# Iancic/Physically-Based-Ray-Tracer

Measured on AMD Instinct MI355X. Metric: Mrays/s (closest-hit segments + shadow any-hit rays) at 1920x1080, 4 spp, depth 4, higher is better.
Workload: dtype f32; 1 GPU; c4-heightfield1m: 1000000 tris, 1920x1080, 4 spp, depth 4; global_batch=2073600, seq_len=4, parallelism=single-gpu, outputs=device (HBM-resident), frames_in_flight=2, warmup_steps_run=75, hw_queues=4

## Files before the change

### include/prt.h

```cpp
#ifndef PRT_H
#define PRT_H
#include <stdint.h>
#include <stddef.h>

#ifdef __cplusplus
extern "C" {
#endif

#define PRT_ABI_VERSION 10

typedef enum {
    PRT_OK = 0,
    PRT_ERR_INVALID_ARGUMENT = -1,
    PRT_ERR_NO_DEVICE = -2,
    PRT_ERR_HIP = -3,
    PRT_ERR_OUT_OF_MEMORY = -4,
    PRT_ERR_NOT_READY = -5,
    PRT_ERR_UNSUPPORTED = -6
} prt_status;

#define PRT_FLAG_AA          (1u << 0)
#define PRT_FLAG_ACCUMULATE  (1u << 1)
#define PRT_FLAG_GAMMA       (1u << 2)
#define PRT_FLAG_NORMALMAP   (1u << 3)
// ... 128 lines not shown
    float vignette_intensity;
    float vignette_radius;
    float color_grading[4];
} prt_postfx;
int prt_postfx_preset(int32_t preset, prt_postfx* out);
int prt_set_postfx(prt_ctx* ctx, const prt_postfx* pfx);

#define PRT_OUT_DEVICE (1u << 0)
int prt_render(prt_ctx* ctx, const prt_render_params* params, float* avg_rgba, uint32_t* rgb8,
               uint32_t out_flags, prt_stats* stats);
int prt_reset_accumulation(prt_ctx* ctx, int32_t full);
int prt_ray_totals(prt_ctx* ctx, uint64_t* segments, uint64_t* shadow_rays, int32_t reset);
int prt_primary_rays(prt_ctx* ctx, uint64_t* traced, uint64_t* reused, int32_t reset);
int prt_shadow_reuse(prt_ctx* ctx, uint64_t* reused, int32_t reset);
int prt_shadow_dead(prt_ctx* ctx, uint64_t* dead, int32_t reset);

int prt_accumulation_bytes(prt_ctx* ctx, uint64_t* bytes);
int prt_save_accumulation(prt_ctx* ctx, void* blob, uint64_t bytes);
int prt_load_accumulation(prt_ctx* ctx, const void* blob, uint64_t bytes);

#define PRT_SHARD_ID_BYTES 128
int prt_shard_unique_id(uint8_t id[PRT_SHARD_ID_BYTES]);
int prt_shard_init_rccl(prt_ctx* ctx, const uint8_t id[PRT_SHARD_ID_BYTES], int32_t rank, int32_t world,
                        int32_t tile_size);
int prt_shard_attach_rccl(prt_ctx* ctx, void* nccl_comm, int32_t tile_size);
int prt_create_group(const prt_device_desc* devices, int32_t count, int32_t tile_size, prt_ctx** out);
typedef struct {
    int32_t rank, world, tile_size;
    int32_t transport;
} prt_shard_info;
// ... 143 lines not shown
```

### include/prt_renderer.hpp

```cpp
#pragma once
#include <algorithm>
#include <array>
#include <cstdint>
#include <map>
#include <stdexcept>
#include <string>
#include <utility>
#include <vector>

#include "prt.h"

namespace prt {

class Error : public std::runtime_error {
 public:
  Error(int code, const std::string& what) : std::runtime_error(what), code(code) {}
  int code;
};

inline void check(int rc) {
  if (rc != PRT_OK) throw Error(rc, std::string("prt error ") + std::to_string(rc) + ": " + prt_last_error());
}

struct Model {
// ... 285 lines not shown
  void RayTotals(uint64_t* segments, uint64_t* shadow_rays, bool reset = false) const {
    check(prt_ray_totals(ctx_, segments, shadow_rays, reset ? 1 : 0));
  }
  void PrimaryRays(uint64_t* traced, uint64_t* reused, bool reset = false) const {
    check(prt_primary_rays(ctx_, traced, reused, reset ? 1 : 0));
  }
  uint64_t ShadowReuse(bool reset = false) const {
    uint64_t reused = 0;
    check(prt_shadow_reuse(ctx_, &reused, reset ? 1 : 0));
    return reused;
  }
  uint64_t ShadowDead(bool reset = false) const {
    uint64_t dead = 0;
    check(prt_shadow_dead(ctx_, &dead, reset ? 1 : 0));
    return dead;
  }

  void Aov(std::vector<float>& albedo, std::vector<float>& normal_depth) {
    albedo.assign(4 * (size_t)width_ * height_, 0.0f);
    normal_depth.assign(4 * (size_t)width_ * height_, 0.0f);
    const prt_postfx pf = camera.PostFx(isPostProcessed);
    check(prt_set_postfx(ctx_, &pf));
    check(prt_render_aov(ctx_, width_, height_, NORMALMAPPED ? PRT_FLAG_NORMALMAP : 0u, albedo.data(),
                         normal_depth.data(), 0u));
  }
  static prt_denoise_params DenoiseDefaults() {
    prt_denoise_params p{};
    check(prt_denoise_defaults(&p));
    return p;
  }
// ... 176 lines not shown
```

### physically-based-ray-tracer_amd/csrc/prt_api_render.cpp

```cpp
#include <hip/hip_runtime.h>

#include <algorithm>
#include <cstdio>
#include <cstdlib>
#include <cstring>
#include <string>
#include <vector>

#include "prt_ctx.h"

using namespace prt;
using namespace prt::host;

namespace {

int check_params(const prt_render_params* p) {
  if (!p) return fail(PRT_ERR_INVALID_ARGUMENT, "params is NULL");
  if (p->width <= 0 || p->height <= 0 || p->width > 16384 || p->height > 16384)
    return fail(PRT_ERR_INVALID_ARGUMENT, "bad resolution");
  if (p->spp < 0) return fail(PRT_ERR_INVALID_ARGUMENT, "spp < 0");
  if ((p->flags & PRT_FLAG_AA) && (p->spp % 2) != 0)
    return fail(PRT_ERR_INVALID_ARGUMENT, "with PRT_FLAG_AA spp must be even (2 paths per reference frame)");
  if (p->bounces < 0 || p->bounces > 16) return fail(PRT_ERR_INVALID_ARGUMENT, "bounces must be in [0,16]");
  if (p->render_mode < 0 || p->render_mode > 6) return fail(PRT_ERR_INVALID_ARGUMENT, "bad render_mode");
// ... 172 lines not shown
    A.frame_index = p->frame_index + f0;
    A.frames = Fb;
    const uint64_t nb = per * (uint64_t)Fb;
    float4* frames = flight_frames(c, fl).as<float4>();
    rc = ensure_wave(ws0, (uint32_t)nb, p->bounces, P.ext(), P.merge(), !P.defer());
    if (rc) return rc;
    ws0.wb.base = 0;
    ws0.wb.coop_tail = P.coop_tail ? 1 : 0;
    ws0.wb.tl = tl;
    ws0.wb.phit = ws0.phit.as<float4>();
    ws0.wb.pitems = (uint32_t)per;
    ws0.wb.pmode = kPrimTrace;
    ws0.wb.lvis = nullptr;
    ws0.wb.lslot = iters + 1;
    ws0.wb.dead = P.dead;
    if (P.preuse && nb > 0) {
      const PrimKey key = prim_key(c, S, M);
      const uint64_t px = tile_image_pixels(M);
      if (ws0.pvalid && std::memcmp(&ws0.pkey, &key, sizeof(key)) == 0) {
        ws0.wb.pmode = kPrimReuse;
        c->prim_reused += px * (uint64_t)Fb;
        if (P.lreuse) {
          float lp[18];
          std::memcpy(lp, S.ppos, sizeof(S.ppos));
          std::memcpy(lp + 12, S.dpos, sizeof(S.dpos));
          std::memcpy(lp + 15, S.spos, sizeof(S.spos));
          if (!(ws0.lvalid && ws0.lgen == ws0.pgen && std::memcmp(lp, ws0.lpos, sizeof(lp)) == 0)) {
            ws0.lvalid = false;
            HIP_TRY(hipMemsetAsync(ws0.lvis.p, 0, sizeof(uint2) * (size_t)per, st));
            ws0.lgen = ws0.pgen;
            std::memcpy(ws0.lpos, lp, sizeof(lp));
            ws0.lvalid = true;
          }
          ws0.wb.lvis = ws0.lvis.as<uint2>();
        }
      } else {
        ws0.wb.pmode = kPrimDense;
        ws0.pgen++;
        ws0.pkey = key;
        ws0.pvalid = false;
        c->prim_traced += px;
        c->prim_reused += px * (uint64_t)(Fb - 1);
      }
    }
    {
      const size_t qw = (size_t)(iters + 2) * 2 * kNSub * kCtrStride;
      const size_t fbase = (size_t)(kMaxIters + 2) * 2 * kNSub * kCtrStride;
      const size_t fw = (size_t)(iters + 2) * 2 * kParts * kCtrStride;
      HIP_TRY(launch_clear2(Lw, ws0.wb.ctr, (uint32_t)qw, ws0.wb.ctr + fbase, (uint32_t)fw));
    }
    if (P.ext() && S.has_diel) HIP_TRY(hipMemsetAsync(ws0.wb.dst, 0, 4ull * ws0.wb.n, st));
    WaveBufs wb = ws0.wb;
    if (P.defer()) point_planes(wb, ws0.planes, (uint32_t)nb, iters);
    HIP_TRY(launch_wave_init(Lw, S, A, M, wb, frames));
    const bool lrec = wb.pmode == kPrimReuse && wb.lvis != nullptr;
    for (uint32_t it = 0; it <= iters; it++)
      HIP_TRY(launch_wave2_iter(Lw, S, A, M, wb, frames, timers ? &c->wt : nullptr, P, lrec, it));
    if (ws0.wb.pmode == kPrimDense) ws0.pvalid = true;
    if (last && want_stats) HIP_TRY(hipEventRecord(c->ev[1], st));
    float4* acc_prev = nullptr;
    if (post && last) {
      const size_t np = (size_t)p->width * p->height;
      if (!avg_dev) { HIP_TRY(c->avg.ensure(np * 16)); avg_dev = c->avg.as<float4>(); }
      if (c->pfx.aberration != 0) { HIP_TRY(c->accprev.ensure(np * 16)); acc_prev = c->accprev.as<float4>(); }
    }
    if (acc_after) HIP_TRY(hipStreamWaitEvent(st, acc_after, 0));
    HIP_TRY(launch_accumulate(L, M, Fb, p->flags, frames, c->acc.as<float4>(), c->nsamp.as<int32_t>(),
                              c->dist.as<float>(), avg_dev, post ? nullptr : rgb8_dev, tiles_dev, acc_prev,
                              ws0.wb.ctr, iters, ray_totals_dev(c)));
    if (post && last) {
      const float4* acc_new = (p->flags & PRT_FLAG_ACCUMULATE) ? c->acc.as<float4>() : avg_dev;
      HIP_TRY(launch_postfx(L, post_params(c, p->width, p->height), acc_new, acc_prev, c->nsamp.as<int32_t>(),
// ... 389 lines not shown

int prt_primary_rays(prt_ctx* c, uint64_t* traced, uint64_t* reused, int32_t reset) {
  if (!c || !traced || !reused) return fail(PRT_ERR_INVALID_ARGUMENT, "bad primary ray counter arguments");
  uint64_t t = c->prim_traced, r = c->prim_reused;
  if (reset) c->prim_traced = c->prim_reused = 0;
  for (prt_ctx* m : c->members) {
    t += m->prim_traced;
    r += m->prim_reused;
    if (reset) m->prim_traced = m->prim_reused = 0;
  }
  *traced = t;
  *reused = r;
  return PRT_OK;
}

int prt_shadow_reuse(prt_ctx* c, uint64_t* reused, int32_t reset) {
  if (!c || !reused) return fail(PRT_ERR_INVALID_ARGUMENT, "bad shadow reuse counter arguments");
  PRT_JOIN(c);
  std::vector<prt_ctx*> all{c};
  all.insert(all.end(), c->members.begin(), c->members.end());
  uint64_t n = 0;
  for (prt_ctx* m : all) {
    HIP_TRY(hipSetDevice(m->device));
    unsigned long long h = 0;
    void* dev = ray_totals_dev(m) + 1;
    HIP_TRY(hipMemcpyAsync(&h, dev, sizeof(h), hipMemcpyDeviceToHost, m->stream));
    if (reset) HIP_TRY(hipMemsetAsync(dev, 0, sizeof(h), m->stream));
    HIP_TRY(hipStreamSynchronize(m->stream));
    n += h;
  }
// ... 180 lines not shown
```

### physically-based-ray-tracer_amd/csrc/prt_ctx.h

```cpp
#pragma once
#include <hip/hip_runtime.h>

#include <memory>
#include <string>
#include <utility>
#include <vector>

#include "../../include/prt.h"
#include "prt_blas_refit_gpu.h"
#include "prt_launch.h"
#include "prt_rccl.h"
#include "prt_refit.h"
#include "prt_skin_gpu.h"
#include "prt_tlas_worker.h"

namespace prt::host {

int fail(int code, const std::string& msg);
std::string& last_error();

#define HIP_TRY(expr)                                                                        \
  do {                                                                                       \
    hipError_t e_ = (expr);                                                                  \
    if (e_ != hipSuccess)                                                                    \
// ... 155 lines not shown
  prt_postfx pfx{};
  DevBuf accprev;
  DevBuf acc, nsamp, dist;
  int32_t accW = 0, accH = 0;
  DevBuf frames, avg, rgb8, counters, hits, tl;
  hipEvent_t ev[3] = {nullptr, nullptr, nullptr};
  prt::host::WaveState ws;
  prt::WaveTimers wt = {};
  uint32_t last_iters = 0;
  bool last_defer = false;
  bool last_timers = false;
  uint64_t last_paths = 0;
  uint64_t carry_segments = 0, carry_shadow = 0;
  uint64_t scene_epoch = 0, inst_epoch = 0;
  uint64_t prim_traced = 0, prim_reused = 0;
  int32_t sh_kind = 0;
  int32_t sh_rank = 0, sh_world = 1, sh_tile = 32;
  ncclComm_t comm = nullptr;
  bool own_comm = false;
  std::vector<prt_ctx*> members;
  DevBuf shtiles, gathered;
  hipEvent_t sh_ev = nullptr;
  bool layout_checked = false;
  int32_t inflight = 1;
  prt::host::Flight fl[prt::host::kMaxFlights];
  int32_t next_fl = 0, last_fl = -1;
  hipEvent_t fl_fork = nullptr;
  DevBuf aov_hits, aov_alb, aov_nd;
  DevBuf dn_in[3], dn_geo, dn_pp[2], dn_out, dn_rgb8;
  hipEvent_t dn_ev[2 + PRT_DENOISE_TIMINGS] = {};
// ... 64 lines not shown
```

### physically-based-ray-tracer_amd/csrc/prt_defer.hip

```cpp
#include "prt_shade2.h"

namespace prt {

template <bool I0>
__global__ void __launch_bounds__(kBlock, I0 ? 4 : 1) k_shade2d(SceneDev S, TraceArgs A, TileMap M, WaveBufs B, uint32_t iter) {
  shade2_body<false, I0, true>(S, A, M, B, iter);
}

__device__ __forceinline__ V3 resolve_path(const SceneDev& S, const WaveBufs& B, uint32_t item, uint32_t first,
                                           uint32_t last, uint32_t rl, uint32_t fl) {
  V3 L = resolve_segment(S, B, (size_t)last * B.n + item, rl, fl);
  for (uint32_t k = last; k > first; k--) {
    const size_t e = (size_t)(k - 1u) * B.n + item;
    const V3 Rk = resolve_segment(S, B, e, B.rinfo[e], fl);
    const float4 Tk = B.T[e];
    L = Rk + L * v3(Tk.x, Tk.y, Tk.z);
  }
  return L;
}
__device__ __forceinline__ uint32_t path_end(const WaveBufs& B, uint32_t item, uint32_t iters, uint32_t it, uint32_t& r) {
  while (((r >> 16) & 3u) == kStNeeCont && it + 1u < iters) r = B.rinfo[(size_t)(++it) * B.n + item];
  return it;
}
template <bool LEARN>
// ... 9 lines not shown
    }
    const uint32_t e1 = path_end(B, item, iters, 0u, r);
    const V3 L1 = resolve_path(S, B, item, 0u, e1, r, fl);
    V3 L = L1;
    if (fl & kAA) {
      if (!(r & kRiQueued) || e1 + 1u >= iters) continue;
      r = B.rinfo[(size_t)(e1 + 1u) * B.n + item];
      const uint32_t e2 = path_end(B, item, iters, e1 + 1u, r);
      L = resolve_path(S, B, item, e1 + 1u, e2, r, fl);
    }
    const V3 res = pixel_value(L1, L, fl);
    out[item] = make_float4(res.x, res.y, res.z, B.s1[item].w);
  }
}

void launch_shade2d(hipStream_t s, unsigned grid, const SceneDev& S, const TraceArgs& A, const TileMap& M,
                    const WaveBufs& B, uint32_t it, bool i0) {
  if (i0) hipLaunchKernelGGL(k_shade2d<true>, dim3(grid), dim3(kBlock), 0, s, S, A, M, B, it);
  else hipLaunchKernelGGL(k_shade2d<false>, dim3(grid), dim3(kBlock), 0, s, S, A, M, B, it);
}
void launch_resolve_pass(hipStream_t s, unsigned grid, const SceneDev& S, const TraceArgs& A, const WaveBufs& B,
                         uint32_t iters, float4* out, bool learn) {
  if (learn) hipLaunchKernelGGL(k_resolve_pass<true>, dim3(grid), dim3(kBlock), 0, s, S, A, B, iters, out);
  else hipLaunchKernelGGL(k_resolve_pass<false>, dim3(grid), dim3(kBlock), 0, s, S, A, B, iters, out);
}

}
```

### physically-based-ray-tracer_amd/csrc/prt_launch.h

```cpp
#pragma once
#include <hip/hip_runtime.h>

#include <cstddef>

#include "prt_kernels.h"
#include "prt_plan.h"
#include "prt_post.h"
#include "prt_traverse8.h"

namespace prt {

struct Counters {
  unsigned long long segments, shadow;
};
struct HitOut {
  float t, u, v;
  uint32_t prim, inst;
};
struct LaunchCfg {
  hipStream_t stream;
  int occ;
  uint32_t groups = 1;
};

// ... 46 lines not shown
void lane_stats_dump();
#endif
constexpr int kTlWaves = 256 * 4 * 8;
struct WaveTimers {
  hipEvent_t ev[4 * (kMaxIters + 1)];
  uint32_t iters;
};

hipError_t launch_wave_init(const LaunchCfg& c, const SceneDev& S, const TraceArgs& A, const TileMap& M,
                            const WaveBufs& B, float4* out);
hipError_t launch_wave2_iter(const LaunchCfg& c, const SceneDev& S, const TraceArgs& A, const TileMap& M,
                             const WaveBufs& B, float4* out, WaveTimers* tm, const WavePlan& P, bool lrec,
                             uint32_t it);
void launch_shade2d(hipStream_t s, unsigned grid, const SceneDev& S, const TraceArgs& A, const TileMap& M,
                    const WaveBufs& B, uint32_t it, bool i0);
void launch_resolve_pass(hipStream_t s, unsigned grid, const SceneDev& S, const TraceArgs& A, const WaveBufs& B,
                         uint32_t iters, float4* out, bool learn);
hipError_t launch_clear2(const LaunchCfg& c, uint32_t* a, uint32_t na, uint32_t* b, uint32_t nb);
hipError_t launch_accumulate(const LaunchCfg& c, const TileMap& M, int32_t frames, uint32_t flags, const float4* fr,
                             float4* acc, int32_t* nsamp, float* dist, float4* avg, uint32_t* rgb8, float4* tiles,
                             float4* acc_prev, const uint32_t* ctr, uint32_t iters, Counters* totals);
hipError_t launch_postfx(const LaunchCfg& c, const PostDev& P, const float4* acc_new, const float4* acc_old,
                         const int32_t* nsamp, const float4* avg, uint32_t* rgb8);
hipError_t launch_untile(const LaunchCfg& c, int32_t W, int32_t H, int32_t ts, int32_t world, uint32_t per_rank,
                         const float4* gathered, float4* avg, uint32_t* rgb8, const PostDev* post);
struct InstSrc;
constexpr uint32_t kSpillTraceBlocks = 256u * 4u * 4u;
constexpr int kSpillTraceStack = 18;
hipError_t launch_refit(hipStream_t s, const InstSrc* src, int32_t n, InstDev* out);
hipError_t launch_wait_host(hipStream_t s, uint32_t* flag, uint32_t* err, double seconds);
// ... 9 lines not shown
```

### physically-based-ray-tracer_amd/csrc/prt_plan.h

```cpp
#pragma once
#include <algorithm>
#include <cassert>
#include <cstddef>
#include <cstdint>
#include <cstdlib>
#include <cstring>

#include "../../include/prt.h"

namespace prt {

constexpr uint32_t kNSub = 32;
constexpr uint32_t kCtrStride = 32;
constexpr uint32_t kParts = 8;
constexpr int kMaxIters = 128;
enum : int32_t { kPrimTrace = 0, kPrimDense = 1, kPrimReuse = 2 };

constexpr uint64_t kMaxPassItems = 1ull << 27;
constexpr uint64_t kMaxMergedPassItems = 1ull << 26;

inline bool debug_queues_on() { return std::getenv("PRT_DEBUG_QUEUES") != nullptr; }
struct Tunables {
  int32_t merge = -1;
  bool defer = true;
  uint64_t defer_budget = 4096ull << 20;
  bool primary_reuse = true;
  bool shadow_reuse = true;
  uint32_t dead_shadow = 2;
  uint64_t max_items = 0;
  bool coop_tail = true;
  bool debug_queues = false;
  int32_t fail_rank = -1;
  bool fail_all = false;
};
inline Tunables read_tunables() {
  Tunables t;
  auto off = [](const char* name) {
    const char* e = std::getenv(name);
    return e && std::atoi(e) == 0;
  };
  if (const char* e = std::getenv("PRT_MERGE")) t.merge = std::atoi(e) != 0 ? 1 : 0;
  t.defer = !off("PRT_DEFER_RESOLVE");
  if (const char* e = std::getenv("PRT_DEFER_BUDGET_MB")) t.defer_budget = std::strtoull(e, nullptr, 10) << 20;
  t.primary_reuse = !off("PRT_PRIMARY_REUSE");
  t.shadow_reuse = !off("PRT_SHADOW_REUSE");
  if (const char* e = std::getenv("PRT_DEAD_SHADOW")) {
    const int v = std::atoi(e);
    t.dead_shadow = v == 0 ? 0u : (v == 1 ? 1u : 2u);
  }
  if (const char* e = std::getenv("PRT_MAX_ITEMS")) t.max_items = std::max<uint64_t>(std::strtoull(e, nullptr, 10), 1);
  t.coop_tail = !off("PRT_TAIL");
  t.debug_queues = debug_queues_on();
  if (const char* e = std::getenv("PRT_FAIL_RENDER"); e && *e) {
    t.fail_all = std::strcmp(e, "all") == 0;
    t.fail_rank = std::max(std::atoi(e), -1);
  }
  return t;
}

constexpr size_t round256(size_t bytes) { return (bytes + 255) & ~size_t(255); }

constexpr size_t kCtrWords = (size_t)(kMaxIters + 2) * 2 * (kNSub + kParts) * kCtrStride;
constexpr uint32_t shadow_per_item(bool merge) { return merge ? 8u : 5u; }

#define PRT_WAVE_ARRAYS(X)                                                                                      \
  X(seed, 4, n, true) X(info, 4, n, true) X(rinfo, 4, ns, true) X(ro, 16, n, true) X(rd, 16, n, true)          \
// ... 53 lines not shown
  const uint32_t paths = (flags & PRT_FLAG_AA) ? 2u : 1u;
  if (merge && paths == 2 && bounces > 0) return 2u * (uint32_t)bounces - 1u;
  if (!dielectric) return paths * (uint32_t)bounces;
  return bounces > 8 ? 0xFFFFFFFFu : paths * ((1u << bounces) - 1u);
}

enum class Pipeline { Plain, PlainDeferred, Merged, Ext, Debug };
struct WavePlan {
  Pipeline pipeline = Pipeline::Plain;
  uint32_t iters = 0;
  int32_t F = 0, fmax = 1, npass = 1, F0 = 0;
  uint64_t per = 0;
  bool preuse = false, lreuse = false;
  uint32_t dead = 2;
  bool coop_tail = true;
  bool timeline = false;
  bool ext() const { return pipeline == Pipeline::Ext; }
  bool merge() const { return pipeline == Pipeline::Merged; }
  bool defer() const { return pipeline == Pipeline::PlainDeferred; }
  uint32_t items0() const { return (uint32_t)(per * (uint64_t)F0); }
};

inline int plan_render(int32_t render_mode, uint32_t flags, int32_t bounces, int32_t spp, uint64_t per, bool area,
                       bool diel, const Tunables& t, WavePlan& P, const char*& err) {
  P = WavePlan{};
  if (per > kMaxPassItems) {
    err = "more than 2^27 pixels in one frame of one shard";
    return PRT_ERR_UNSUPPORTED;
  }
  const bool aa = (flags & PRT_FLAG_AA) != 0;
// ... 13 lines not shown
  P.F0 = std::min(F, P.fmax);
  P.iters = wave_iters(diel, bounces, flags, merge);
  if (P.iters > (uint32_t)kMaxIters) {
    err = diel ? "dielectric path trees exceed the wavefront iteration limit (lower bounces)"
               : "too many wavefront iterations";
    return PRT_ERR_UNSUPPORTED;
  }
  const bool defer = plain && !merge && P.items0() != 0 && t.defer &&
                     plane_layout(P.items0(), P.iters).bytes <= t.defer_budget;
  P.pipeline = merge ? Pipeline::Merged : !mode0 ? Pipeline::Debug : ext ? Pipeline::Ext
               : defer ? Pipeline::PlainDeferred : Pipeline::Plain;
  P.preuse = plain && t.primary_reuse && per > 0 && F > 0;
  P.lreuse = P.preuse && t.shadow_reuse;
  P.dead = t.dead_shadow;
  P.coop_tail = t.coop_tail;
  P.timeline = t.debug_queues;
  return PRT_OK;
}

enum class Kernel {
  None,
  Trace2, Trace2Dense,
  Res2d, Res2dLearn, Res2md, Res2mdLearn,
  ResolvePass, ResolvePassLearn,
  Miss2, Miss2Ext, ResMiss2, ResMiss2Ext,
  Shade2, Shade2Learn, Shade2Ext, Shade2Debug,
  Shade2d, Shade2dLearn, Shade2m, Shade2mLearn,
};
struct Schedule {
  Kernel trace, resolve, shade;
};
inline Schedule wave_schedule(Pipeline p, bool lrec, int32_t pmode, uint32_t it, uint32_t iters) {
  const bool plainish = p == Pipeline::Plain || p == Pipeline::PlainDeferred;
  assert(!lrec || pmode == kPrimReuse);
  assert((plainish || p == Pipeline::Merged) || (pmode == kPrimTrace && !lrec));
  const bool learn_res = lrec && it == 1, learn_shade = lrec && it == 0;
  Schedule s{Kernel::Trace2, Kernel::None, Kernel::None};
  if (it == 0 && pmode == kPrimDense) s.trace = Kernel::Trace2Dense;
  else if (it == 0 && pmode == kPrimReuse && plainish) s.trace = Kernel::None;
  switch (p) {
    case Pipeline::Plain:
      if (it > 0) s.resolve = learn_res ? Kernel::Res2dLearn : Kernel::Res2d;
      s.shade = learn_shade ? Kernel::Shade2Learn : Kernel::Shade2;
      break;
    case Pipeline::PlainDeferred:
      if (it == iters) s.resolve = lrec ? Kernel::ResolvePassLearn : Kernel::ResolvePass;
      s.shade = learn_shade ? Kernel::Shade2dLearn : Kernel::Shade2d;
      break;
    case Pipeline::Merged:
      if (it > 0) s.resolve = learn_res ? Kernel::Res2mdLearn : Kernel::Res2md;
      s.shade = learn_shade ? Kernel::Shade2mLearn : Kernel::Shade2m;
      break;
    case Pipeline::Ext:
      s.resolve = it > 0 ? Kernel::ResMiss2Ext : Kernel::Miss2Ext;
      s.shade = Kernel::Shade2Ext;
      break;
    case Pipeline::Debug:
      s.resolve = it > 0 ? Kernel::ResMiss2 : Kernel::Miss2;
      s.shade = Kernel::Shade2Debug;
      break;
  }
  if (it >= iters) s.shade = Kernel::None;
  return s;
}

}
```

### physically-based-ray-tracer_amd/csrc/prt_wave2.hip

```cpp
#include <cstdio>

#include "prt_launch.h"
#include "prt_path.h"
#include "prt_persist.h"
#include "prt_queue.h"

namespace prt {

#ifdef PRT_LANE_STATS
__device__ unsigned long long g_lane_stats[(kMaxIters + 2) * 32];
void lane_stats_dump() {
  static unsigned long long h[(kMaxIters + 2) * 32];
  if (hipMemcpyFromSymbol(h, HIP_SYMBOL(g_lane_stats), sizeof(h)) != hipSuccess) return;
  for (int i = 0; i < kMaxIters + 2; i++) {
    const unsigned long long* r = h + 32 * i;
    if (!r[31]) continue;
    std::fprintf(stderr, "prt: lanestats %d", i);
    for (int k = 0; k < 32; k++) std::fprintf(stderr, " %llu", r[k]);
    std::fprintf(stderr, "\n");
  }
  static const unsigned long long z[(kMaxIters + 2) * 32] = {};
  (void)hipMemcpyToSymbol(HIP_SYMBOL(g_lane_stats), z, sizeof(z));
}
#endif
// ... 454 lines not shown
  return g < kNSub ? kNSub : g - g % kNSub;
}

hipError_t launch_wave2_iter(const LaunchCfg& c, const SceneDev& S, const TraceArgs& A, const TileMap& M,
                             const WaveBufs& B, float4* out, WaveTimers* tm, const WavePlan& P, bool lrec,
                             uint32_t it) {
  if (B.n == 0) return hipSuccess;
  const unsigned gprod = producer_blocks(c);
#ifndef PRT_SHADE_GRID
  const unsigned gshade = B.n >= (1u << 21) ? 4u * gprod : gprod;
#else
  static_assert(PRT_SHADE_GRID % kNSub == 0, "PRT_SHADE_GRID must be a multiple of kNSub");
  const unsigned gshade = PRT_SHADE_GRID;
#endif
  const uint32_t iters = P.iters;
  const Schedule k = wave_schedule(P.pipeline, lrec, B.pmode, it, iters);
  if (tm) (void)hipEventRecord(tm->ev[4 * it + 0], c.stream);
  WaveBufs Bt = B, Bs = B;
  if (P.defer()) {
    if (it > 0) Bt.vis = B.vis + (size_t)(it - 1u) * B.n;
    const size_t o = (size_t)it * B.n;
    Bs.rinfo += o; Bs.ne += o; Bs.nb += o; Bs.nk += o; Bs.vis += o; Bs.T += o;
  }
  if (k.trace == Kernel::Trace2Dense) launch_trace2_t<true>(c, S, Bt, it, iters);
  else if (k.trace == Kernel::Trace2) launch_trace2_t<false>(c, S, Bt, it, iters);
  if (tm) (void)hipEventRecord(tm->ev[4 * it + 1], c.stream);
#ifndef PRT_RES_GRID
  const unsigned gres = gprod;
#else
  const unsigned gres = PRT_RES_GRID;
#endif
// ... 5 lines not shown
    case Kernel::Res2dLearn: PRT_LAUNCH(k_res2d<true>, gdense, S, A, B, out); break;
    case Kernel::Res2d: PRT_LAUNCH(k_res2d<false>, gdense, S, A, B, out); break;
    case Kernel::ResolvePassLearn: launch_resolve_pass(c.stream, gdense, S, A, B, iters, out, true); break;
    case Kernel::ResolvePass: launch_resolve_pass(c.stream, gdense, S, A, B, iters, out, false); break;
    case Kernel::ResMiss2Ext: PRT_LAUNCH(k_resmiss2<true>, gres, S, A, B, it, iters, 1u, out); break;
    case Kernel::ResMiss2: PRT_LAUNCH(k_resmiss2<false>, gres, S, A, B, it, iters, 1u, out); break;
    case Kernel::Miss2Ext: PRT_LAUNCH(k_miss2<true>, gprod, S, A, B, it); break;
    case Kernel::Miss2: PRT_LAUNCH(k_miss2<false>, gprod, S, A, B, it); break;
    default: assert(k.resolve == Kernel::None);
  }
  switch (k.shade) {
    case Kernel::Shade2mLearn: PRT_LAUNCH(k_shade2m<true>, gshade, S, A, M, B, it); break;
    case Kernel::Shade2m: PRT_LAUNCH(k_shade2m<false>, gshade, S, A, M, B, it); break;
    case Kernel::Shade2Debug: PRT_LAUNCH(k_shade2_debug, gprod, S, A, M, B, it); break;
    case Kernel::Shade2Ext: PRT_LAUNCH(k_shade2<true>, gshade, S, A, M, B, it); break;
    case Kernel::Shade2dLearn: launch_shade2d(c.stream, gshade, S, A, M, Bs, it, true); break;
    case Kernel::Shade2d: launch_shade2d(c.stream, gshade, S, A, M, Bs, it, false); break;
    case Kernel::Shade2Learn: PRT_LAUNCH((k_shade2<false, true>), gshade, S, A, M, B, it); break;
    case Kernel::Shade2: PRT_LAUNCH(k_shade2<false>, gshade, S, A, M, B, it); break;
    default: assert(k.shade == Kernel::None);
  }
#undef PRT_LAUNCH
  if (tm) tm->iters = iters + 1;
  return hipGetLastError();
}

hipError_t launch_wave_init(const LaunchCfg& c, const SceneDev& S, const TraceArgs& A, const TileMap& M,
                            const WaveBufs& B, float4* out) {
  hipLaunchKernelGGL(k_wave_init, dim3(producer_blocks(c)), dim3(kBlock), 0, c.stream, S, A, M, B, out);
  return hipGetLastError();
// ... 4 lines not shown
```

### physically-based-ray-tracer_amd/prt/_lib.py

```python
from __future__ import annotations

import ctypes as C
import os

HERE = os.path.dirname(os.path.abspath(__file__))
LIBPATH = os.environ.get("PRT_LIBPATH") or os.path.join(HERE, "libprt.so")

PRT_OK = 0
ABI_VERSION = 10
FLAG_AA, FLAG_ACCUMULATE, FLAG_GAMMA, FLAG_NORMALMAP, FLAG_SKYBOX, FLAG_LIGHTED, FLAG_STOCHASTIC = (1 << i for i in range(7))
FLAGS_DEFAULT = 0x7F
OUT_DEVICE = 1
IN_DEVICE = 1
OUT_TIMED = 2
DENOISE_TIMINGS = 10
BUILDER_HOST_SAH, BUILDER_GPU_LBVH, BUILDER_HOST_SBVH, BUILDER_GPU_PLOC = 0, 1, 2, 3

MODE_BRDF, MODE_BASECOLOR, MODE_GEOMETRYNORMAL, MODE_SHADINGNORMAL, MODE_METAL, MODE_ROUGHNESS, MODE_EMISSIVE = range(7)

EXPORTS = [
    "prt_abi_version", "prt_last_error", "prt_device_count", "prt_create", "prt_destroy", "prt_set_stream",
    "prt_set_textures", "prt_set_meshes", "prt_set_instances", "prt_set_lights", "prt_set_sky", "prt_set_camera",
    "prt_camera_look_at", "prt_postfx_preset", "prt_set_postfx", "prt_render", "prt_reset_accumulation", "prt_tile_buffer_pixels", "prt_tile_pixel_map",
    "prt_render_tiles",
    "prt_untile", "prt_trace_primary", "prt_intersect", "prt_occluded", "prt_brdf_probe", "prt_get_scene_info", "prt_set_bvh_builder",
    "prt_set_instance_materials", "prt_set_area_lights", "prt_shard_unique_id", "prt_shard_init_rccl",
    "prt_shard_attach_rccl", "prt_create_group", "prt_get_shard_info", "prt_accumulation_bytes",
    "prt_save_accumulation", "prt_load_accumulation", "prt_ray_totals", "prt_set_frames_in_flight", "prt_finish",
    "prt_render_aov", "prt_denoise_defaults", "prt_denoise", "prt_denoise_timings",
    "prt_reproject_defaults", "prt_reproject", "prt_primary_rays", "prt_shadow_reuse",
    "prt_shadow_dead",
    "prt_render_aov_ids", "prt_instance_motion", "prt_reproject_motion",
    "prt_temporal_defaults", "prt_reproject_moments", "prt_denoise_variance_defaults", "prt_denoise_variance",
    "prt_update_mesh", "prt_read_blas", "prt_read_blas_tris",
    "prt_snapshot_mesh", "prt_render_aov_deform", "prt_reproject_deform",
    "prt_set_mesh_skin", "prt_skin_mesh",
]
SHARD_ID_BYTES = 128
SHARD_NONE, SHARD_RCCL, SHARD_GROUP = 0, 1, 2

MAT_TEXTURED, MAT_DIELECTRIC, MAT_MIRROR = 0, 1, 2


class PrtError(RuntimeError):
    pass


class DeviceDesc(C.Structure):
    _fields_ = [("device", C.c_int32), ("flags", C.c_uint32)]


class Texture(C.Structure):
# ... 118 lines not shown
        "prt_set_lights": ([vp, C.POINTER(Lights)], C.c_int),
        "prt_set_sky": ([vp, vp, i32, i32], C.c_int),
        "prt_set_camera": ([vp, C.POINTER(CameraDesc)], C.c_int),
        "prt_camera_look_at": ([vp, vp, C.c_float, C.POINTER(CameraDesc)], C.c_int),
        "prt_postfx_preset": ([i32, C.POINTER(PostFx)], C.c_int),
        "prt_set_postfx": ([vp, C.POINTER(PostFx)], C.c_int),
        "prt_render": ([vp, C.POINTER(RenderParams), vp, vp, u32, C.POINTER(Stats)], C.c_int),
        "prt_reset_accumulation": ([vp, i32], C.c_int),
        "prt_accumulation_bytes": ([vp, C.POINTER(C.c_uint64)], C.c_int),
        "prt_save_accumulation": ([vp, vp, C.c_uint64], C.c_int),
        "prt_load_accumulation": ([vp, vp, C.c_uint64], C.c_int),
        "prt_ray_totals": ([vp, C.POINTER(C.c_uint64), C.POINTER(C.c_uint64), C.c_int32], C.c_int),
        "prt_primary_rays": ([vp, C.POINTER(C.c_uint64), C.POINTER(C.c_uint64), C.c_int32], C.c_int),
        "prt_shadow_reuse": ([vp, C.POINTER(C.c_uint64), C.c_int32], C.c_int),
        "prt_shadow_dead": ([vp, C.POINTER(C.c_uint64), C.c_int32], C.c_int),
        "prt_tile_buffer_pixels": ([i32, i32, i32, i32, C.POINTER(C.c_int64)], C.c_int),
        "prt_tile_pixel_map": ([i32, i32, i32, i32, i32, C.c_void_p], C.c_int),
        "prt_render_tiles": ([vp, C.POINTER(RenderParams), i32, i32, i32, vp, C.POINTER(Stats)], C.c_int),
        "prt_untile": ([vp, vp, i32, i32, i32, i32, vp, vp], C.c_int),
        "prt_trace_primary": ([vp, i32, i32, vp, u32, C.POINTER(Stats)], C.c_int),
        "prt_intersect": ([vp, i32, vp, vp, vp, vp], C.c_int),
        "prt_occluded": ([vp, i32, vp, vp, vp, vp], C.c_int),
        "prt_brdf_probe": ([vp, i32, i32, vp, vp], C.c_int),
        "prt_get_scene_info": ([vp, C.POINTER(SceneInfo)], C.c_int),
        "prt_set_bvh_builder": ([vp, i32], C.c_int),
        "prt_set_instance_materials": ([vp, vp, i32], C.c_int),
        "prt_set_area_lights": ([vp, C.POINTER(AreaLight), i32], C.c_int),
        "prt_shard_unique_id": ([vp], C.c_int),
        "prt_shard_init_rccl": ([vp, vp, i32, i32, i32], C.c_int),
        "prt_shard_attach_rccl": ([vp, vp, i32], C.c_int),
# ... 9 lines not shown
        "prt_render_aov_ids": ([vp, i32, i32, u32, vp, vp, vp, u32], C.c_int),
        "prt_instance_motion": ([vp, vp, i32, vp], C.c_int),
        "prt_reproject_motion": ([vp, C.POINTER(ReprojectParams), i32, i32, C.POINTER(CameraDesc), vp, vp, vp,
                                  C.POINTER(CameraDesc), vp, vp, vp, vp, i32, vp, vp, u32], C.c_int),
        "prt_temporal_defaults": ([C.POINTER(TemporalParams)], C.c_int),
        "prt_reproject_moments": ([vp, C.POINTER(TemporalParams), i32, i32, C.POINTER(CameraDesc), vp, vp, vp,
                                   C.POINTER(CameraDesc), vp, vp, vp, vp, i32, vp, vp, vp, vp, u32], C.c_int),
        "prt_render_aov_deform": ([vp, i32, i32, u32, vp, vp, vp, vp, u32], C.c_int),
        "prt_reproject_deform": ([vp, C.POINTER(TemporalParams), i32, i32, C.POINTER(CameraDesc), vp, vp, vp,
                                  C.POINTER(CameraDesc), vp, vp, vp, vp, i32, vp, vp, vp, vp, vp, vp, u32], C.c_int),
        "prt_denoise_variance_defaults": ([C.POINTER(DenoiseVarianceParams)], C.c_int),
        "prt_denoise_variance": ([vp, C.POINTER(DenoiseVarianceParams), i32, i32, vp, vp, vp, vp, vp, vp, vp, u32],
                                 C.c_int),
    }
    for name, (args, res) in sig.items():
        f = getattr(L, name)
        f.argtypes = args
        f.restype = res
    if L.prt_abi_version() != ABI_VERSION:
        raise PrtError(f"{LIBPATH}: ABI {L.prt_abi_version()} != {ABI_VERSION} (stale build: rerun __graft_entry__.build())")
    _lib = L
    return L


def check(rc: int) -> None:
    if rc != PRT_OK:
        msg = load().prt_last_error()
        raise PrtError(f"prt error {rc}: {msg.decode() if msg else ''}")
```

### physically-based-ray-tracer_amd/prt/renderer.py

```python
from __future__ import annotations

import ctypes as C
from dataclasses import dataclass, field

import numpy as np

from . import _lib
from ._lib import check

F32 = np.float32


def _f32(a):
    return np.ascontiguousarray(a, dtype=np.float32)


def _ptr(a):
    return a.ctypes.data if isinstance(a, np.ndarray) else a


def _images(n, device_out, timed=False, f32=(), u32=(), outs=()):
    of = (_lib.OUT_DEVICE if device_out else 0) | (_lib.OUT_TIMED if timed else 0)
    if device_out:
        return list(f32), list(u32), [o[0] for o in outs], of
# ... 414 lines not shown
    def primary_rays(self, reset=False):
        tr, re_ = C.c_uint64(), C.c_uint64()
        check(self.L.prt_primary_rays(self.h, C.byref(tr), C.byref(re_), 1 if reset else 0))
        return int(tr.value), int(re_.value)

    def shadow_reuse(self, reset=False):
        n = C.c_uint64()
        check(self.L.prt_shadow_reuse(self.h, C.byref(n), 1 if reset else 0))
        return int(n.value)

    def shadow_dead(self, reset=False):
        n = C.c_uint64()
        check(self.L.prt_shadow_dead(self.h, C.byref(n), 1 if reset else 0))
        return int(n.value)

    def save_accumulation(self) -> bytes:
        n = C.c_uint64()
        check(self.L.prt_accumulation_bytes(self.h, C.byref(n)))
        if n.value == 0:
            return b""
        buf = (C.c_uint8 * n.value)()
        check(self.L.prt_save_accumulation(self.h, buf, n.value))
        return bytes(buf)

    def load_accumulation(self, blob: bytes):
        buf = (C.c_uint8 * len(blob)).from_buffer_copy(blob)
        check(self.L.prt_load_accumulation(self.h, buf, len(blob)))

    def trace_primary(self, width, height):
        hits = np.zeros(width * height, dtype=[("t", F32), ("u", F32), ("v", F32), ("prim", np.uint32),
# ... 350 lines not shown
```

Baseline: 6220 Mrays/s.

## Fuse wave-init into the first deferred shade pass when primary hits are reused

Adds a k_shade2d_init kernel that does per-pixel path setup (seed, jitter, primary ray, miss handling) inside the first shade iteration of the PlainDeferred pipeline when primary hits and light visibility are reused. When that path applies, the separate wave-init launch is skipped. The goal is to drop one full-screen kernel launch and its round trip of per-item state through global memory. It adds a new code path that is on by default but can be disabled with PRT_FUSED_INIT, falls back when the lvis buffer was just cleared, and adds a counter API.

```diff
diff --git a/include/prt.h b/include/prt.h
--- a/include/prt.h
+++ b/include/prt.h
@@ -166,6 +166,7 @@
 int prt_primary_rays(prt_ctx* ctx, uint64_t* traced, uint64_t* reused, int32_t reset);
 int prt_shadow_reuse(prt_ctx* ctx, uint64_t* reused, int32_t reset);
 int prt_shadow_dead(prt_ctx* ctx, uint64_t* dead, int32_t reset);
+int prt_fused_init_passes(prt_ctx* ctx, uint64_t* passes, int32_t reset);
 
 int prt_accumulation_bytes(prt_ctx* ctx, uint64_t* bytes);
 int prt_save_accumulation(prt_ctx* ctx, void* blob, uint64_t bytes);
diff --git a/include/prt_renderer.hpp b/include/prt_renderer.hpp
--- a/include/prt_renderer.hpp
+++ b/include/prt_renderer.hpp
@@ -323,6 +323,11 @@
     uint64_t dead = 0;
     check(prt_shadow_dead(ctx_, &dead, reset ? 1 : 0));
     return dead;
+  }
+  uint64_t FusedInitPasses(bool reset = false) const {
+    uint64_t passes = 0;
+    check(prt_fused_init_passes(ctx_, &passes, reset ? 1 : 0));
+    return passes;
   }
 
   void Aov(std::vector<float>& albedo, std::vector<float>& normal_depth) {
diff --git a/physically-based-ray-tracer_amd/csrc/prt_api_render.cpp b/physically-based-ray-tracer_amd/csrc/prt_api_render.cpp
--- a/physically-based-ray-tracer_amd/csrc/prt_api_render.cpp
+++ b/physically-based-ray-tracer_amd/csrc/prt_api_render.cpp
@@ -210,6 +210,7 @@
     ws0.wb.lvis = nullptr;
     ws0.wb.lslot = iters + 1;
     ws0.wb.dead = P.dead;
+    bool lcleared = false;
     if (P.preuse && nb > 0) {
       const PrimKey key = prim_key(c, S, M);
       const uint64_t px = tile_image_pixels(M);
@@ -223,6 +224,7 @@
           std::memcpy(lp + 15, S.spos, sizeof(S.spos));
           if (!(ws0.lvalid && ws0.lgen == ws0.pgen && std::memcmp(lp, ws0.lpos, sizeof(lp)) == 0)) {
             ws0.lvalid = false;
+            lcleared = true;
             HIP_TRY(hipMemsetAsync(ws0.lvis.p, 0, sizeof(uint2) * (size_t)per, st));
             ws0.lgen = ws0.pgen;
             std::memcpy(ws0.lpos, lp, sizeof(lp));
@@ -248,10 +250,14 @@
     if (P.ext() && S.has_diel) HIP_TRY(hipMemsetAsync(ws0.wb.dst, 0, 4ull * ws0.wb.n, st));
     WaveBufs wb = ws0.wb;
     if (P.defer()) point_planes(wb, ws0.planes, (uint32_t)nb, iters);
-    HIP_TRY(launch_wave_init(Lw, S, A, M, wb, frames));
     const bool lrec = wb.pmode == kPrimReuse && wb.lvis != nullptr;
+    WavePlan Pp = P;
+    Pp.fused_init = P.fused_init && !lcleared;
+    if (wave_init(Pp.pipeline, lrec, wb.pmode, iters, Pp.fused_init) == Kernel::WaveInit)
+      HIP_TRY(launch_wave_init(Lw, S, A, M, wb, frames));
+    else if (nb > 0) c->fused_passes++;
     for (uint32_t it = 0; it <= iters; it++)
-      HIP_TRY(launch_wave2_iter(Lw, S, A, M, wb, frames, timers ? &c->wt : nullptr, P, lrec, it));
+      HIP_TRY(launch_wave2_iter(Lw, S, A, M, wb, frames, timers ? &c->wt : nullptr, Pp, lrec, it));
     if (ws0.wb.pmode == kPrimDense) ws0.pvalid = true;
     if (last && want_stats) HIP_TRY(hipEventRecord(c->ev[1], st));
     float4* acc_prev = nullptr;
@@ -671,6 +677,18 @@
   return PRT_OK;
 }
 
+int prt_fused_init_passes(prt_ctx* c, uint64_t* passes, int32_t reset) {
+  if (!c || !passes) return fail(PRT_ERR_INVALID_ARGUMENT, "bad fused-init counter arguments");
+  uint64_t n = c->fused_passes;
+  if (reset) c->fused_passes = 0;
+  for (prt_ctx* m : c->members) {
+    n += m->fused_passes;
+    if (reset) m->fused_passes = 0;
+  }
+  *passes = n;
+  return PRT_OK;
+}
+
 int prt_shadow_reuse(prt_ctx* c, uint64_t* reused, int32_t reset) {
   if (!c || !reused) return fail(PRT_ERR_INVALID_ARGUMENT, "bad shadow reuse counter arguments");
   PRT_JOIN(c);
diff --git a/physically-based-ray-tracer_amd/csrc/prt_ctx.h b/physically-based-ray-tracer_amd/csrc/prt_ctx.h
--- a/physically-based-ray-tracer_amd/csrc/prt_ctx.h
+++ b/physically-based-ray-tracer_amd/csrc/prt_ctx.h
@@ -193,6 +193,7 @@
   uint64_t carry_segments = 0, carry_shadow = 0;
   uint64_t scene_epoch = 0, inst_epoch = 0;
   uint64_t prim_traced = 0, prim_reused = 0;
+  uint64_t fused_passes = 0;
   int32_t sh_kind = 0;
   int32_t sh_rank = 0, sh_world = 1, sh_tile = 32;
   ncclComm_t comm = nullptr;
diff --git a/physically-based-ray-tracer_amd/csrc/prt_defer.hip b/physically-based-ray-tracer_amd/csrc/prt_defer.hip
--- a/physically-based-ray-tracer_amd/csrc/prt_defer.hip
+++ b/physically-based-ray-tracer_amd/csrc/prt_defer.hip
@@ -47,10 +47,101 @@
   }
 }
 
+__global__ void __launch_bounds__(kBlock, 4) k_shade2d_init(SceneDev S, TraceArgs A, TileMap M, WaveBufs B,
+                                                            uint32_t iter, float4* __restrict__ out) {
+  const Shade2ArgsPtr args = (Shade2ArgsPtr)__builtin_amdgcn_kernarg_segment_ptr();
+  if (args->iter != iter || args->B.n != B.n || blockDim.x != kBlock) {
+    if (blockIdx.x == 0 && threadIdx.x == 0) atomicOr(S.diag + 1, 1u);
+    return;
+  }
+  __shared__ uint32_t sm[8];
+  const uint32_t sub = blockIdx.x % kNSub;
+  uint32_t* shcnt = qcounter(B.ctr, 0, 1, sub);
+  uint32_t* ncnt = qcounter(B.ctr, 1, 0, sub);
+  uint32_t* shq = B.shq + (size_t)sub * B.scap;
+  const uint32_t fl = A.flags;
+  uint32_t f_n = 0, r_n = 0;
+  float4 hh_n = make_float4(kFar, 0.0f, 0.0f, 0.0f);
+  uint2 lv_n = make_uint2(0u, 0u);
+  auto prefetch = [&](uint32_t cc) {
+    const uint32_t ii = cc * kBlock + threadIdx.x;
+    if (ii < B.n) {
+      const uint32_t gi = B.base + ii;
+      f_n = gi / M.items;
+      r_n = gi % M.items;
+      hh_n = B.phit[r_n];
+      lv_n = B.lvis[r_n];
+    }
+  };
+  prefetch(blockIdx.x);
+  uint32_t queued0 = 0;
+  for (uint32_t c = blockIdx.x; c * kBlock < B.n; c += gridDim.x) {
+    Shade2ArgsPtr ka = args;
+    asm volatile("" : "+s"(ka));
+    const SceneDev& Sc = *(const SceneDev*)&ka->S;
+    const WaveBufs& Bc = *(const WaveBufs*)&ka->B;
+    const uint32_t item = c * kBlock + threadIdx.x;
+    uint32_t seed = 0, nr = 0;
+    Asked q;
+    q.cached = true;
+    int kind = 0;
+    float4 hh = make_float4(kFar, 0.0f, 0.0f, 0.0f);
+    float4 ro_c = make_float4(0.0f, 0.0f, 0.0f, 0.0f), rd_c = ro_c;
+    bool active = false;
+    if (item < Bc.n) {
+      int32_t x, y;
+      active = item_pixel(M, r_n, x, y);
+      if (active) {
+        hh = hh_n;
+        const uint2 lv = lv_n;
+        const uint32_t p = (uint32_t)(y * A.W + x);
+        seed = init_seed(A.seed + p + (uint32_t)A.W * (uint32_t)A.H * (A.frame_index + f_n));
+        if (fl & kAA) {
+          const float jx = random_float(seed), jy = random_float(seed);
+          Bc.jit[item] = make_float2(jx, jy);
+        }
+        const Ray r1 = primary_ray(Sc, (float)x, (float)y, A.W, A.H);
+        ro_c = make_float4(r1.O.x, r1.O.y, r1.O.z, 0.0f);
+        rd_c = make_float4(r1.D.x, r1.D.y, r1.D.z, 0.0f);
+        Bc.s1[item].w = hh.x;
+        if (hh.x >= kFar) {
+          shade_miss(Sc, Bc, fl, item, rd_c);
+          Bc.seed[item] = seed;
+        } else {
+          kind = nee_kind(fl, seed);
+          nr = (uint32_t)nee_rays(kind);
+          lvis_split(lv, kind, q.ask, q.vis0);
+        }
+      } else {
+        out[item] = make_float4(0.0f, 0.0f, 0.0f, kFar);
+        Bc.rinfo[item] = 0u;
+      }
+    }
+    queued0 += (uint32_t)__popcll(__ballot(active));
+    prefetch(c + gridDim.x);
+    q.s0 = block_append_skip(shcnt, (uint32_t)__popc(q.ask), qcounter(B.ctr, B.lslot, 1, sub), lvis_total(S),
+                             nr - (uint32_t)__popc(q.ask), sm);
+    ShadedHit h = {kStMiss << 16, 0u, false};
+    if (nr) h = shade_hit<false>(Sc, A, Bc, item, item, (size_t)item, ro_c, rd_c, hh, kind, nr, 0u, seed, q, shq);
+    bool next = h.cont();
+    if (active) {
+      if (!next) next = start_path2(Sc, A, M, Bc, item, 0u);
+      Bc.rinfo[item] = h.rinfo | ((uint32_t)kind << 20) | (next ? kRiQueued : 0u) | kResFresh | (q.ask ? kRiLearn : 0u);
+    }
+    const uint32_t slot = block_append(ncnt, next ? 1u : 0u, sm);
+    if (next) Bc.q1[sub * Bc.qcap + slot] = item;
+  }
+  if (lane_id() == 0 && queued0) atomicAdd(qcounter(B.ctr, 0, 0, sub), queued0);
+}
+
 void launch_shade2d(hipStream_t s, unsigned grid, const SceneDev& S, const TraceArgs& A, const TileMap& M,
                     const WaveBufs& B, uint32_t it, bool i0) {
   if (i0) hipLaunchKernelGGL(k_shade2d<true>, dim3(grid), dim3(kBlock), 0, s, S, A, M, B, it);
   else hipLaunchKernelGGL(k_shade2d<false>, dim3(grid), dim3(kBlock), 0, s, S, A, M, B, it);
+}
+void launch_shade2d_init(hipStream_t s, unsigned grid, const SceneDev& S, const TraceArgs& A, const TileMap& M,
+                         const WaveBufs& B, float4* out) {
+  hipLaunchKernelGGL(k_shade2d_init, dim3(grid), dim3(kBlock), 0, s, S, A, M, B, 0u, out);
 }
 void launch_resolve_pass(hipStream_t s, unsigned grid, const SceneDev& S, const TraceArgs& A, const WaveBufs& B,
                          uint32_t iters, float4* out, bool learn) {
diff --git a/physically-based-ray-tracer_amd/csrc/prt_launch.h b/physically-based-ray-tracer_amd/csrc/prt_launch.h
--- a/physically-based-ray-tracer_amd/csrc/prt_launch.h
+++ b/physically-based-ray-tracer_amd/csrc/prt_launch.h
@@ -84,6 +84,8 @@
                              uint32_t it);
 void launch_shade2d(hipStream_t s, unsigned grid, const SceneDev& S, const TraceArgs& A, const TileMap& M,
                     const WaveBufs& B, uint32_t it, bool i0);
+void launch_shade2d_init(hipStream_t s, unsigned grid, const SceneDev& S, const TraceArgs& A, const TileMap& M,
+                         const WaveBufs& B, float4* out);
 void launch_resolve_pass(hipStream_t s, unsigned grid, const SceneDev& S, const TraceArgs& A, const WaveBufs& B,
                          uint32_t iters, float4* out, bool learn);
 hipError_t launch_clear2(const LaunchCfg& c, uint32_t* a, uint32_t na, uint32_t* b, uint32_t nb);
diff --git a/physically-based-ray-tracer_amd/csrc/prt_plan.h b/physically-based-ray-tracer_amd/csrc/prt_plan.h
--- a/physically-based-ray-tracer_amd/csrc/prt_plan.h
+++ b/physically-based-ray-tracer_amd/csrc/prt_plan.h
@@ -29,6 +29,7 @@
   uint32_t dead_shadow = 2;
   uint64_t max_items = 0;
   bool coop_tail = true;
+  bool fused_init = true;
   bool debug_queues = false;
   int32_t fail_rank = -1;
   bool fail_all = false;
@@ -50,6 +51,7 @@
   }
   if (const char* e = std::getenv("PRT_MAX_ITEMS")) t.max_items = std::max<uint64_t>(std::strtoull(e, nullptr, 10), 1);
   t.coop_tail = !off("PRT_TAIL");
+  t.fused_init = !off("PRT_FUSED_INIT");
   t.debug_queues = debug_queues_on();
   if (const char* e = std::getenv("PRT_FAIL_RENDER"); e && *e) {
     t.fail_all = std::strcmp(e, "all") == 0;
@@ -133,6 +135,7 @@
   bool preuse = false, lreuse = false;
   uint32_t dead = 2;
   bool coop_tail = true;
+  bool fused_init = true;
   bool timeline = false;
   bool ext() const { return pipeline == Pipeline::Ext; }
   bool merge() const { return pipeline == Pipeline::Merged; }
@@ -176,23 +179,26 @@
   P.lreuse = P.preuse && t.shadow_reuse;
   P.dead = t.dead_shadow;
   P.coop_tail = t.coop_tail;
+  P.fused_init = t.fused_init;
   P.timeline = t.debug_queues;
   return PRT_OK;
 }
 
 enum class Kernel {
   None,
+  WaveInit,
   Trace2, Trace2Dense,
   Res2d, Res2dLearn, Res2md, Res2mdLearn,
   ResolvePass, ResolvePassLearn,
   Miss2, Miss2Ext, ResMiss2, ResMiss2Ext,
   Shade2, Shade2Learn, Shade2Ext, Shade2Debug,
   Shade2d, Shade2dLearn, Shade2m, Shade2mLearn,
+  Shade2dInit,
 };
 struct Schedule {
   Kernel trace, resolve, shade;
 };
-inline Schedule wave_schedule(Pipeline p, bool lrec, int32_t pmode, uint32_t it, uint32_t iters) {
+inline Schedule wave_schedule(Pipeline p, bool lrec, int32_t pmode, uint32_t it, uint32_t iters, bool fused = false) {
   const bool plainish = p == Pipeline::Plain || p == Pipeline::PlainDeferred;
   assert(!lrec || pmode == kPrimReuse);
   assert((plainish || p == Pipeline::Merged) || (pmode == kPrimTrace && !lrec));
@@ -207,7 +213,7 @@
       break;
     case Pipeline::PlainDeferred:
       if (it == iters) s.resolve = lrec ? Kernel::ResolvePassLearn : Kernel::ResolvePass;
-      s.shade = learn_shade ? Kernel::Shade2dLearn : Kernel::Shade2d;
+      s.shade = learn_shade ? (fused ? Kernel::Shade2dInit : Kernel::Shade2dLearn) : Kernel::Shade2d;
       break;
     case Pipeline::Merged:
       if (it > 0) s.resolve = learn_res ? Kernel::Res2mdLearn : Kernel::Res2md;
@@ -225,5 +231,8 @@
   if (it >= iters) s.shade = Kernel::None;
   return s;
 }
-
-}
+inline Kernel wave_init(Pipeline p, bool lrec, int32_t pmode, uint32_t iters, bool fused) {
+  return wave_schedule(p, lrec, pmode, 0, iters, fused).shade == Kernel::Shade2dInit ? Kernel::None : Kernel::WaveInit;
+}
+
+}
diff --git a/physically-based-ray-tracer_amd/csrc/prt_wave2.hip b/physically-based-ray-tracer_amd/csrc/prt_wave2.hip
--- a/physically-based-ray-tracer_amd/csrc/prt_wave2.hip
+++ b/physically-based-ray-tracer_amd/csrc/prt_wave2.hip
@@ -492,7 +492,7 @@
   const unsigned gshade = PRT_SHADE_GRID;
 #endif
   const uint32_t iters = P.iters;
-  const Schedule k = wave_schedule(P.pipeline, lrec, B.pmode, it, iters);
+  const Schedule k = wave_schedule(P.pipeline, lrec, B.pmode, it, iters, P.fused_init);
   if (tm) (void)hipEventRecord(tm->ev[4 * it + 0], c.stream);
   WaveBufs Bt = B, Bs = B;
   if (P.defer()) {
@@ -528,6 +528,7 @@
     case Kernel::Shade2m: PRT_LAUNCH(k_shade2m<false>, gshade, S, A, M, B, it); break;
     case Kernel::Shade2Debug: PRT_LAUNCH(k_shade2_debug, gprod, S, A, M, B, it); break;
     case Kernel::Shade2Ext: PRT_LAUNCH(k_shade2<true>, gshade, S, A, M, B, it); break;
+    case Kernel::Shade2dInit: launch_shade2d_init(c.stream, gshade, S, A, M, Bs, out); break;
     case Kernel::Shade2dLearn: launch_shade2d(c.stream, gshade, S, A, M, Bs, it, true); break;
     case Kernel::Shade2d: launch_shade2d(c.stream, gshade, S, A, M, Bs, it, false); break;
     case Kernel::Shade2Learn: PRT_LAUNCH((k_shade2<false, true>), gshade, S, A, M, B, it); break;
diff --git a/physically-based-ray-tracer_amd/prt/_lib.py b/physically-based-ray-tracer_amd/prt/_lib.py
--- a/physically-based-ray-tracer_amd/prt/_lib.py
+++ b/physically-based-ray-tracer_amd/prt/_lib.py
@@ -29,13 +29,14 @@
     "prt_save_accumulation", "prt_load_accumulation", "prt_ray_totals", "prt_set_frames_in_flight", "prt_finish",
     "prt_render_aov", "prt_denoise_defaults", "prt_denoise", "prt_denoise_timings",
     "prt_reproject_defaults", "prt_reproject", "prt_primary_rays", "prt_shadow_reuse",
-    "prt_shadow_dead",
+    "prt_shadow_dead", "prt_fused_init_passes",
     "prt_render_aov_ids", "prt_instance_motion", "prt_reproject_motion",
     "prt_temporal_defaults", "prt_reproject_moments", "prt_denoise_variance_defaults", "prt_denoise_variance",
     "prt_update_mesh", "prt_read_blas", "prt_read_blas_tris",
     "prt_snapshot_mesh", "prt_render_aov_deform", "prt_reproject_deform",
     "prt_set_mesh_skin", "prt_skin_mesh",
 ]
+SINCE_ABI_10 = {"prt_fused_init_passes"}
 SHARD_ID_BYTES = 128
 SHARD_NONE, SHARD_RCCL, SHARD_GROUP = 0, 1, 2
 
@@ -184,6 +185,7 @@
         "prt_primary_rays": ([vp, C.POINTER(C.c_uint64), C.POINTER(C.c_uint64), C.c_int32], C.c_int),
         "prt_shadow_reuse": ([vp, C.POINTER(C.c_uint64), C.c_int32], C.c_int),
         "prt_shadow_dead": ([vp, C.POINTER(C.c_uint64), C.c_int32], C.c_int),
+        "prt_fused_init_passes": ([vp, C.POINTER(C.c_uint64), C.c_int32], C.c_int),
         "prt_tile_buffer_pixels": ([i32, i32, i32, i32, C.POINTER(C.c_int64)], C.c_int),
         "prt_tile_pixel_map": ([i32, i32, i32, i32, i32, C.c_void_p], C.c_int),
         "prt_render_tiles": ([vp, C.POINTER(RenderParams), i32, i32, i32, vp, C.POINTER(Stats)], C.c_int),
@@ -223,6 +225,8 @@
                                  C.c_int),
     }
     for name, (args, res) in sig.items():
+        if name in SINCE_ABI_10 and LIBPATH != os.path.join(HERE, "libprt.so") and not hasattr(L, name):
+            continue
         f = getattr(L, name)
         f.argtypes = args
         f.restype = res
diff --git a/physically-based-ray-tracer_amd/prt/renderer.py b/physically-based-ray-tracer_amd/prt/renderer.py
--- a/physically-based-ray-tracer_amd/prt/renderer.py
+++ b/physically-based-ray-tracer_amd/prt/renderer.py
@@ -452,6 +452,11 @@
         check(self.L.prt_shadow_dead(self.h, C.byref(n), 1 if reset else 0))
         return int(n.value)
 
+    def fused_init_passes(self, reset=False):
+        n = C.c_uint64()
+        check(self.L.prt_fused_init_passes(self.h, C.byref(n), 1 if reset else 0))
+        return int(n.value)
+
     def save_accumulation(self) -> bytes:
         n = C.c_uint64()
         check(self.L.prt_accumulation_bytes(self.h, C.byref(n)))
```

Measured after the change: 6292 Mrays/s, median of 6. 1.2% higher.
